# wildjames/lfit_python

Measured on AMD Instinct MI355X. Metric: walker ln_prob evals/sec (300-pt phase, complex BS) at 1/2/4/8 MI355X, higher is better.
Workload: dtype f64

## Files before the change

lfit_python_amd/csrc/lfg.hip:

```cpp
#include <hip/hip_runtime.h>
#include <atomic>
#include <stdint.h>
#include <stdlib.h>

#include <type_traits>

#include "lfg.h"
#include "lfg_device.hpp"
#include "lfg_tables.hpp"

using namespace lfg;

#include "lfg_diag.hpp"

namespace {

constexpr int SETUP_BLOCK = 64;
#ifndef LFG_ELEM_BLOCK
#define LFG_ELEM_BLOCK 64
#endif
constexpr int ELEM_BLOCK = LFG_ELEM_BLOCK;
#ifndef LFG_ELEM_IPL
#define LFG_ELEM_IPL 1
#endif
#ifndef ELEM_MINW
#define ELEM_MINW 4
#endif
constexpr int WT_DISC = 0, WT_TD = NDISC_R, WT_BS = 24, WT_N = WT_BS + NBS;
constexpr int NU_WDD = (NWD + NDISC) / 2, NELU = NU_WDD + NBS;
__device__ __forceinline__ int uitem(int g) { return (g * 37) % NU_WDD; }
__device__ __forceinline__ int uslot(int u) { return (u * 473) % NU_WDD; }
static_assert(NU_WDD == 700 && (37 * 473) % 700 == 1, "sweep permutation inverse");
__device__ __forceinline__ double2 mirror_ab(double2 ab)
{
// ... 422 lines not shown
        G[G_GP_RWD] = rwd;
        G[G_GP_OK] = !ok ? 0.0 : (pend ? 2.0 : (isfinite(B[3]) ? 1.0 : 0.0));
    }
    LFG_CY(3, t, tl);
}

#ifndef LFG_NOLICM_TU
__global__ __launch_bounds__(SETUP_BLOCK) void k_setup(SetupArgs A)
{
    setup_any(A, blockIdx.x * SETUP_BLOCK + threadIdx.x);
}
#endif

#ifdef LFG_COUNT_ITERS
__device__ unsigned long long g_iter_dbg[64];

#endif
constexpr int U_WD = NWD / 2, U_DISC = NDISC / 2, U_BS = NBS, U_DON = NDONOR / 4;
constexpr int NUNIQ = U_WD + U_DISC + U_BS + U_DON;
constexpr int U_MAIN = U_WD + U_DISC + U_DON;

__device__ __forceinline__ int wd_ring_of(int u)
{
    int ir = int(sqrt(u * 0.5));
    if (2 * (ir + 1) * (ir + 1) <= u) ++ir;
    if (2 * ir * ir > u) --ir;
    return ir;
}

__device__ inline double wd_ring_weight(int ir, double ul) { return fma(kWdA[ir], 1.0 - ul, kWdB[ir] * ul); }

template <typename GPtr>
__device__ inline double disc_boundary(int i, GPtr G)
{
    const double rin = G[G_RWD];
    const double r = rin + i * ((G[G_RDISC] - rin) / NDISC_R);
    const double ex = 2.0 - G[G_DEXP];
    return (fabs(ex) < 1e-10) ? log(r) : pow(r, ex) / ex;
}

template <typename GPtr>
__device__ inline double disc_ring_weight(int ir, GPtr G)
{
    return (TWO_PI / NDISC_AZ) * (disc_boundary(ir + 1, G) - disc_boundary(ir, G));
}

template <typename GPtr>
__device__ inline double bs_weight(int j, GPtr G)
{
    const double uk = (j + 0.5) * (G[G_UMAX] / NBS);
// ... 13 lines not shown
    const int* bstatusC;
    const double* priorC;
    const double* qC;
    const double* zfC;
    double* prior;
    double* q;
    double* zf;
    int* bstatus;
    int E, ndim;
    const double* lprior;
    SetupArgs S[2];
    int nspec;
    int nspecblk;
};

struct ElemOut {
    double2* abw;
    double2* abs;
    double* don;
    double* wtd;
    double* wbs;
};

template <typename GPtr>
__device__ __forceinline__ void ring_weight_lane(int rb, GPtr G, double* __restrict__ wtd)
{
    const double P = disc_boundary(rb, G);
    const int lane = int(threadIdx.x) & 63, l0 = lane - rb;
    const double Pn = __shfl(P, min(lane + 1, l0 + NDISC_R), 64);
    const double Pt = __shfl(P, l0 + NDISC_R, 64);
    if (rb < NDISC_R) wtd[rb] = (TWO_PI / NDISC_AZ) * (Pn - P);
    if (rb == 0) wtd[NDISC_R] = TWO_PI * (Pt - P);
}

template <typename GPtr, typename Sink>
__device__ __forceinline__ void element_item_to(int v, GPtr G, Sink& K);

struct MemSink {
    const ElemOut& O;
    __device__ __forceinline__ void mark() {}
    __device__ __forceinline__ void wd_disc(int u, double a, double b) { O.abw[uslot(u)] = make_double2(a, b); }
    __device__ __forceinline__ void spot(int j, double a, double b, double w)
    {
        O.abs[j] = make_double2(a, b);
        O.wbs[j] = w;
    }
    __device__ __forceinline__ void donor(int uu, double vx, double vy, double vz, double cen, double hw)
    {
        double* D = O.don + uu * DON_STRIDE;
        D[0] = vx;
        D[1] = vy;
        D[2] = vz;
        D[3] = cen;
        D[4] = hw;
    }
// ... 67 lines not shown
        const double ig = rsqrt(gx * gx + gy * gy + gz * gz);
        const double nx = gx * ig, ny = gy * ig, nz = gz * ig;
        const double dA = r * r * kDonOmega[it] / (nx * dx + ny * dy + nz * dz);
        const double vx = dA * nx, vy = dA * ny, vz = dA * nz;
        const double srho = s * sqrt(vx * vx + vy * vy);
        const double kap = (srho > 0.0) ? -c * vz / srho : (c * vz > 0.0 ? -2.0 : 2.0);
        const double cen = -atan2(vy, vx) * (1.0 / TWO_PI), hw = acos(fmin(fmax(kap, -1.0), 1.0)) * (1.0 / TWO_PI);
        K.mark();
        K.donor(uu, vx, vy, vz, cen, hw);
        return;
    }

    double Px, Py, Pz;
    if (u < U_WD) {
        const int ir = wd_ring_of(u);
        const double rc = kWdRc[ir], mu0 = kWdMu0[ir];
        const double cp = kWdCos[u], sp = kWdSin[u];
        const double rw = G[G_RWD];
        Px = rw * (-rc * sp * c + mu0 * s);
        Py = rw * (rc * cp);
        Pz = rw * (rc * sp * s + mu0 * c);
    } else if (u < U_WD + U_DISC) {
        const int uu = u - U_WD;
        const int ir = uu / (NDISC_AZ / 2), j = uu - ir * (NDISC_AZ / 2);
        const double rin = G[G_RWD];
        const double rc = rin + (ir + 0.5) * ((G[G_RDISC] - rin) / NDISC_R);
        Px = rc * kDiscCos[j];
        Py = rc * kDiscSin[j];
        Pz = 0.0;
    } else {
        const int j = u - U_MAIN;
        const double uk = (j + 0.5) * (G[G_UMAX] / NBS);
        const double off = G[G_L] * (uk - G[G_UPK]);
        Px = fma(off, G[G_CAZ], G[G_BSX]);
        Py = fma(off, G[G_SAZ], G[G_BSY]);
        Pz = 0.0;
    }
    double a, b;
#ifdef LFG_COUNT_ITERS
    bool fb = false;
    int nit[3] = {0, 0, 0};
    double gs[2] = {0.0, 0.0};
    element_interval_fast(R, Px, Py, Pz, s, c, G[G_RCAL], G[G_REFF], a, b, &fb, nit, gs);
    {
        const int reg = (u < U_WD) ? 0 : (u < U_WD + U_DISC ? 1 : 2);
        unsigned long long* C = g_iter_dbg + reg * 16;
        for (int i = 0; i < 3; ++i) {
// ... 259 lines not shown
        const uint4 r = draw(L.seed, L.step, L.half, 1, w);
        const double lu = log(u53(r.x, r.y));
        if (lu < L.zfac[w] + v - L.lnp_ens[wg]) {
            double* p = L.pos + size_t(wg) * L.ndim;
            const double* qi = L.qprop + size_t(w) * L.ndim;
            for (int d = 0; d < L.ndim; ++d) p[d] = qi[d];
            L.lnp_ens[wg] = v;
            if (L.naccept) L.naccept[wg] += 1;
            if (L.accflag) L.accflag[w] = 1;
        } else if (L.accflag) {
            L.accflag[w] = 0;
        }
    }
}

__device__ inline void finish_walker(const LikeArgs& L, int pair, int tid, bool acc1, const double* sq,
                                     const double* sacc1, int* sflag);

__device__ inline void combine_after(const LikeArgs& L, int pair)
{
    if (L.combine) combine_walker(L, pair / L.E);
}

constexpr int LIKE_THREADS = 512;
constexpr int ACC_LDS = 24;
#ifndef LIKE_MINW
#define LIKE_MINW 4
#endif
constexpr int LIKE_TILE = LIKE_THREADS;
constexpr int LIKE_NC = 2 * LIKE_TILE;
#ifndef LFG_WALK
#define LFG_WALK 2
#endif
constexpr double FX_SCALE = 2305843009213693952.0;
constexpr double FX_INV = 1.0 / FX_SCALE;

struct PhaseIndex {
    const double* v;
    const int* cell;
    int m;
    double t0, ginv;
};

__device__ __forceinline__ int cell_of(const PhaseIndex& X, double v)
{
    const double u = (v - X.t0) * X.ginv;
    return u <= 0.0 ? 0 : (u >= double(LIKE_NC) ? LIKE_NC : int(u));
}

template <bool LE>
__device__ __forceinline__ int count_below(const PhaseIndex& X, double x)
{
    int j = X.cell[cell_of(X, x)];
    const int last = X.m - 1;
    bool adv = false;
#pragma unroll
    for (int k = 0; k < LFG_WALK; ++k) {
        const double vj = X.v[min(j, last)];
        adv = (j <= last) & (LE ? (vj <= x) : (vj < x));
        j += adv ? 1 : 0;
    }
    if (adv)
        while (j <= last && (LE ? (X.v[j] <= x) : (X.v[j] < x))) ++j;
    return j;
}

template <int Q>
__device__ __forceinline__ void count_lt_multi(const PhaseIndex& X, const double (&x)[Q], int (&j)[Q])
{
    const int last = X.m - 1;
#pragma unroll
    for (int q = 0; q < Q; ++q) j[q] = X.cell[cell_of(X, x[q])];
    bool adv[Q];
#pragma unroll
    for (int k = 0; k < LFG_WALK; ++k) {
#pragma unroll
        for (int q = 0; q < Q; ++q) {
            const double vj = X.v[min(j[q], last)];
            adv[q] = (j[q] <= last) & (vj < x[q]);
            j[q] += adv[q] ? 1 : 0;
        }
    }
#pragma unroll
    for (int q = 0; q < Q; ++q)
        if (adv[q])
            while (j[q] <= last && X.v[j[q]] < x[q]) ++j[q];
}

template <int Q>
__device__ __forceinline__ void count_le_back_multi(const double* __restrict__ hi, const double (&x)[Q],
                                                    const int (&J)[Q], int (&out)[Q])
{
    bool back[Q];
#pragma unroll
    for (int q = 0; q < Q; ++q) {
        back[q] = (J[q] > 0) & (hi[max(J[q] - 1, 0)] > x[q]);
        out[q] = J[q] - (back[q] ? 1 : 0);
    }
#pragma unroll
    for (int q = 0; q < Q; ++q)
        if (back[q])
            while (out[q] > 0 && hi[out[q] - 1] > x[q]) --out[q];
}

__device__ __forceinline__ int count_le_back(const double* __restrict__ hi, int J, double x)
{
    const bool back = (J > 0) & (hi[max(J - 1, 0)] > x);
    J -= back ? 1 : 0;
    if (back)
        while (J > 0 && hi[J - 1] > x) --J;
    return J;
}

__device__ __forceinline__ PhaseIndex phase_index(const double* v, const int* cell, int m)
{
    const double span = v[m - 1] - v[0];
    return PhaseIndex{v, cell, m, v[0], span > 0.0 ? LIKE_NC / span : 0.0};
}

__device__ __forceinline__ void build_cells(const double* __restrict__ v, int m, int* __restrict__ cell, int tid)
{
    const PhaseIndex X = phase_index(v, cell, m);
    const double t0 = X.t0, ginv = X.ginv;
    auto ci = [&](double x) {
        const double u = (x - t0) * ginv;
        return u < 0.0 ? -1 : (u >= double(LIKE_NC) ? LIKE_NC : int(u));
    };
    if (tid < m) {
        const int g0 = tid ? ci(v[tid - 1]) : -1, g1 = ci(v[tid]);
        for (int g = g0 + 1; g <= g1; ++g) cell[g] = tid;
        if (tid == m - 1)
            for (int g = g1 + 1; g <= LIKE_NC; ++g) cell[g] = m;
    }
}

__device__ __forceinline__ long long to_fx(double x) { return static_cast<long long>(rint(x * FX_SCALE)); }

__device__ __forceinline__ void fx_add(unsigned long long* acc, int p, long long q)
{
    atomicAdd(acc + p, static_cast<unsigned long long>(q));
}

struct Runs {
    int P1, P2, P3, P4;
};

__device__ __forceinline__ Runs element_runs(double a, double b, const PhaseIndex& X, const double* __restrict__ hi)
{
    Runs R;
    R.P2 = count_below<false>(X, a);
    R.P4 = count_below<false>(X, b);
    R.P1 = count_le_back(hi, R.P2, a);
    R.P3 = count_le_back(hi, R.P4, b);
    return R;
}

__device__ __forceinline__ void apply_runs(const Runs& R, double a, double b, double wn, const PhaseIndex& X,
                                           const double* __restrict__ hi, const double* __restrict__ iw,
                                           unsigned long long* acc)
{
    const int P1 = R.P1, P2 = R.P2, P3 = R.P3, P4 = R.P4;
    int e0 = P4, s1 = P4;
    if (P2 < P3) {
        const long long q = to_fx(wn);
        fx_add(acc, P2, q);
        if (P3 < X.m) fx_add(acc, P3, -q);
        e0 = P2;
        s1 = P3;
    }
    for (int r = 0; r < 2; ++r) {
        const int pe = r ? P4 : e0;
        for (int p = r ? s1 : P1; p < pe; ++p) {
            const double ov = fmin(b, hi[p]) - fmax(a, X.v[p]);
            if (ov > 0.0) {
                const long long q = to_fx(wn * ov * iw[p]);
                fx_add(acc, p, q);
                if (p + 1 < X.m) fx_add(acc, p + 1, -q);
            }
        }
    }
}

template <int NI>
__device__ __forceinline__ void apply_runs_batched(const Runs (&R)[NI], const double (&a)[NI], const double (&b)[NI],
                                                   double wn, const PhaseIndex& X, const double* __restrict__ hi,
                                                   const double* __restrict__ iw, unsigned long long* acc)
{
    constexpr int K = 2;
    const int last = X.m - 1;
    int ps[NI][2], pn[NI][2];
    long long q[NI][2][K];
#pragma unroll
    for (int k = 0; k < NI; ++k) {
        const bool whole = R[k].P2 < R[k].P3;
        const int e0 = whole ? R[k].P2 : R[k].P4, s1 = whole ? R[k].P3 : R[k].P4;
        ps[k][0] = R[k].P1;
        pn[k][0] = e0 - R[k].P1;
        ps[k][1] = s1;
        pn[k][1] = R[k].P4 - s1;
#pragma unroll
        for (int e = 0; e < 2; ++e)
#pragma unroll
            for (int i = 0; i < K; ++i) {
                const int p = min(ps[k][e] + i, last);
                const double ov = fmin(b[k], hi[p]) - fmax(a[k], X.v[p]);
                q[k][e][i] = (i < pn[k][e] && ov > 0.0) ? to_fx(wn * ov * iw[p]) : 0;
            }
    }
    const long long qw = to_fx(wn);
#pragma unroll
    for (int k = 0; k < NI; ++k) {
        if (R[k].P2 < R[k].P3) {
            fx_add(acc, R[k].P2, qw);
            if (R[k].P3 < X.m) fx_add(acc, R[k].P3, -qw);
        }
#pragma unroll
        for (int e = 0; e < 2; ++e)
#pragma unroll
            for (int i = 0; i < K; ++i) {
                const int p = ps[k][e] + i;
                if (q[k][e][i] != 0) {
                    fx_add(acc, p, q[k][e][i]);
                    if (p + 1 < X.m) fx_add(acc, p + 1, -q[k][e][i]);
                }
            }
    }
#pragma unroll
    for (int k = 0; k < NI; ++k)
#pragma unroll
        for (int e = 0; e < 2; ++e)
            for (int p = ps[k][e] + K; p < ps[k][e] + pn[k][e]; ++p) {
                const double ov = fmin(b[k], hi[p]) - fmax(a[k], X.v[p]);
                if (ov > 0.0) {
                    const long long qq = to_fx(wn * ov * iw[p]);
                    fx_add(acc, p, qq);
                    if (p + 1 < X.m) fx_add(acc, p + 1, -qq);
                }
            }
}

__device__ __forceinline__ int uring(int u)
{
    if (u >= U_WD) return NWD_RINGS + (u - U_WD) / (NDISC_AZ / 2);
    int r = int(sqrtf(float(u) * 0.5f));
    r += (2 * (r + 1) * (r + 1) <= u) ? 1 : 0;
    r -= (2 * r * r > u) ? 1 : 0;
    return r;
}

__device__ __forceinline__ long long wave_scan_incl(long long v, int lane)
{
    (void)lane;
    v += dpp64<0x111, 0xf>(v);
    v += dpp64<0x112, 0xf>(v);
    v += dpp64<0x114, 0xf>(v);
    v += dpp64<0x118, 0xf>(v);
    v += dpp64<0x142, 0xa>(v);
    v += dpp64<0x143, 0xc>(v);
    return v;
}

__device__ __forceinline__ long long wave_total(long long v)
{
    v = wave_scan_incl(v, 0);
    const int lo = __builtin_amdgcn_readlane(static_cast<int>(v), 63);
    const int hi = __builtin_amdgcn_readlane(static_cast<int>(v >> 32), 63);
    return (static_cast<long long>(hi) << 32) | static_cast<unsigned>(lo);
}

template <int NA>
// ... 1152 lines not shown
    double2* ab;
    double2* sab;
    double* sbw;
    double* sdq;
    unsigned long long* mk;
    long long tspot, tdon, bx, by, bz;

    __device__ __forceinline__ void mark()
    {
#ifdef LFG_PROFILE_PAIR
        if (mk) *mk = __builtin_amdgcn_s_memrealtime();
#endif
    }
    __device__ __forceinline__ void wd_disc(int u, double a, double b)
    {
#ifdef LFG_ABL_SINK_WD
        return;
#endif
        if (dir) {
            ab[uslot(u)] = make_double2(a, b);
            return;
        }
        if (!(a < b)) return;
        const int ir = uring(u);
        const double wn = (u < U_WD) ? wd_ring_weight(ir, ul) * itwd : swt[ir - NWD_RINGS] * (1.0 / swt[NDISC_R]);
        double q[4] = {a, b, -b, -a};
        int J[4], Jb[4];
        count_lt_multi<4>(XW, q, J);
        count_le_back_multi<4>(hi, q, J, Jb);
        unsigned long long* A = ((lane & 1) ? acc2 : acc)[(u < U_WD) ? 0 : 1];
        const Runs RR[2] = {Runs{Jb[0], J[0], Jb[1], J[1]}, Runs{Jb[2], J[2], Jb[3], J[3]}};
        const double aa[2] = {a, -b}, bb[2] = {b, -a};
        apply_runs_batched<2>(RR, aa, bb, wn, XW, hi, iw, A);
    }
    __device__ __forceinline__ void spot(int j, double a, double b, double w)
    {
        sab[j] = make_double2(a, b);
        sbw[j] = w;
        tspot += to_fx(w * PAIR_SPOT_S);
#ifdef LFG_ABL_SINK_SPOT
        if (false) {
#else
        if (!dir && a < b) {
#endif
            const Runs RR[1] = {element_runs(a, b, XW, hi)};
            const double aa[1] = {a}, bb[1] = {b};
            apply_runs_batched<1>(RR, aa, bb, w * PAIR_SPOT_S, XW, hi, iw, acc[2]);
        }
    }
    __device__ __forceinline__ void donor(int uu, double vx0, double vy0, double vz0, double cen0, double hw0)
    {
        double* D = sdq + uu * DON_STRIDE;
        D[0] = vx0;
        D[1] = vy0;
        D[2] = vz0;
        D[3] = cen0;
        D[4] = hw0;
        long long tn = 0;
        int PA[4][2], QA[4][2];
#pragma unroll
        for (int mr = 0; mr < 4; ++mr) {
            const double vy = (mr & 1) ? -vy0 : vy0, vz = (mr & 2) ? -vz0 : vz0;
            const double cen = (mr & 1) ? -cen0 : cen0;
            const double hw = (mr & 2) ? 0.5 - hw0 : hw0;
            tn += to_fx(fmax(-s * vy + c * vz, 0.0) * PAIR_DON_S);
            PA[mr][0] = QA[mr][0] = PA[mr][1] = QA[mr][1] = 0;
#ifdef LFG_ABL_SINK_DON
            continue;
#endif
            if (dir || !(hw > 0.0)) continue;
// ... 505 lines not shown
        amin[1] = fmin(amin[1], W.part[5][k]); bmax[1] = fmax(bmax[1], W.part[6][k]);
        sa = fmin(sa, W.part[2][k]); sb = fmax(sb, W.part[3][k]); vs += W.part[4][k];
    }
    double t0[2], ginv[2];
    for (int t = 0; t < 2; ++t) {
        t0[t] = amin[t];
        ginv[t] = (bmax[t] > amin[t]) ? LONG_FC / (bmax[t] - amin[t]) : 0.0;
    }
    const double st0 = sa, sginv = (sb > sa) ? TCELLS / (sb - sa) : 0.0;
    constexpr double t0d = -0.5, t1d = 0.5, dginv = TCELLS;
    const double itb = 1.0 / (double(static_cast<long long>(stot[0])) * (FX_INV / PAIR_SPOT_S)), ivs = 1.0 / vs;
    if (tid == 0) {
        for (int t = 0; t < 2; ++t) { W.t0[t] = t0[t]; W.ginv[t] = ginv[t]; W.amin[t] = amin[t]; W.bmax[t] = bmax[t]; }
        W.snorm[0] = itb;
        W.snorm[1] = ivs;
        W.snorm[2] = double(static_cast<long long>(stot[1])) * (FX_INV / PAIR_DON_S);
        W.snorm[3] = vs;
        W.shull[0] = fmin(amin[0], amin[1]); W.shull[1] = fmax(bmax[0], bmax[1]); W.shull[2] = sa; W.shull[3] = sb;
        T.dt0 = t0d; T.dginv = dginv; T.st0 = st0; T.sginv = sginv;
    }
    auto wd_entry = [&](int g, double2& ab, int& t, long long& q) {
        ab = abw[g];
        if (!(ab.x < ab.y)) return false;
        const int u = uitem(g), ir = uring(u);
        t = u < U_WD ? 0 : 1;
        q = to_fx(u < U_WD ? wd_ring_weight(ir, ul) * itwd : swt[ir - NWD_RINGS] * (1.0 / swt[NDISC_R]));
        return true;
    };
    for (int g = tid; g < NU_WDD; g += nt) {
        double2 ab;
        int t;
        long long q;
        if (!wd_entry(g, ab, t, q)) continue;
        (void)q;
        atomicAdd(&W.fend[t][long_cell(ab.x, t0[t], ginv[t])], 1);
        atomicAdd(&W.fend[t][long_cell(ab.y, t0[t], ginv[t])], 1);
    }
    {
        double p0, p1;
        bool in0, in1;
        int v0;
        lane_breakpoints(tid, sdq, sab, t0d, t1d, p0, p1, in0, in1, v0);
        long long c0[3] = {0, 0, 0};
        if (tid >= nt - NDONOR) {
            long long q[3];
            donor_q(sdq, tid - (nt - NDONOR), ivs, q[0], q[1], q[2]);
            for (int k = 0; k < 3; ++k) c0[k] = v0 * q[k];
// ... 215 lines not shown
        for (int k = k0; k < k1; ++k) {
            run += q[k];
            q[k] = run;
        }
    }
    if (tid >= 128 && tid < 128 + U_DON) {
        double* dq = sdq + (tid - 128) * DON_STRIDE;
        const long long q0 = to_fx(dq[0] * ivs), q1 = to_fx(dq[1] * ivs), q2 = to_fx(dq[2] * ivs);
        LongV* dl = reinterpret_cast<LongV*>(dq);
        dl[0] = q0;
        dl[1] = q1;
        dl[2] = q2;
    }
    __syncthreads();
    LONG_TSTAMP(6);
}

template <bool GP, bool FOLD = false, bool LONG = false>
__global__ __launch_bounds__(LIKE_THREADS, LIKE_MINW) void k_pair(PairArgs A)
{
    static_assert(!(GP && LONG), "GP trees keep the one-tile layout or the two kernels");
    const LikeArgs& L = A.L;
    const ElemSpec& X = A.X;
    __shared__ double swt[NDISC_R + 1];
    __shared__ double sbw[NBS];
    __shared__ double2 sab[NBS];
    __shared__ double sdq[U_DON * DON_STRIDE];
    __shared__ double sacc1[3];
    __shared__ TileBufs TA;
    __shared__ double sph[LIKE_TILE];
    __shared__ union PairU_ {
        struct {
            unsigned long long X[2][LIKE_TILE + 1];
            int scp[LIKE_NC + 1];
        } s;
        double2 ab[NU_WDD];
    } SU;
    __shared__ unsigned long long sacc[6][LIKE_TILE + 1];
    __shared__ unsigned long long stot[2];
#if !LFG_PAIR_RUNSCAN
    __shared__ long long spart[6][LIKE_THREADS / 64];
#endif
    __shared__ double red[LIKE_THREADS / 64];
    __shared__ int sflagw[LIKE_THREADS / 64];
    __shared__ int sflag[1];
    __shared__ int sjob;
    __shared__ double sq[ACC_LDS];
// ... 123 lines not shown
        if (tid <= m) {
            for (int i = 0; i < 6; ++i) sacc[i][tid] = 0ull;
            SU.s.X[0][tid] = 0ull;
            SU.s.X[1][tid] = 0ull;
        }
#else
        for (int i = 0; i < 6; ++i) sacc[i][tid] = 0ull;
        SU.s.X[0][tid] = 0ull;
        SU.s.X[1][tid] = 0ull;
#endif
    }
    if (tid == 0) {
#if !LFG_PAIR_RUNSCAN
        if constexpr (!LONG) {
            for (int i = 0; i < 6; ++i) sacc[i][nt] = 0ull;
            SU.s.X[0][nt] = 0ull;
            SU.s.X[1][nt] = 0ull;
        }
#endif
        stot[0] = stot[1] = 0ull;
        sjob = (X.nspec > 0 && pair < 2 * A.nbc) ? 8 : 9;
    }
    PAIR_STAMP(19, tid == 0);
    if (st == ST_OK && wv == 7 && lane <= NDISC_R) ring_weight_lane(lane, Gc, swt);
    __syncthreads();
    PAIR_STAMP(16, tid == 0);

    bool dir = LONG;
    if (!LONG)
        for (int k = 0; k < nw; ++k) dir = dir || sflagw[k] != 0;
    if (own) {
        sy[tid] = L.y[o0 + tid];
        if (!GP) sye[tid] = L.ye[o0 + tid];
        if (GP) {
            const double xp = L.x[o0 + tid], dx = xp - (tid ? L.x[o0 + tid - 1] : xp);
            L.gpx[size_t(pair) * L.N + tid] = exp(-(Gc[G_GP_LAM] * dx));
        }
    }
    const bool pend = GP && st == ST_OK && Gc[G_GP_OK] == 2.0;
    auto fold_rows = [&](int l) {
        const int ns = A.jns, h = L.half, hp = 1 - h, nd = L.ndim, r = (ns + nwk - 1) / nwk;
        for (int f = l; f < r * nd; f += 64) {
            const int k = f / nd, d = f - k * nd, j = w + k * nwk;
            if (j < ns) A.fsnap[size_t(j) * nd + d] = A.fpos[(size_t(h) * ns + j) * nd + d];
        }
        if (A.fv) {
            for (int f = l; f < r * nd; f += 64) {
// ... 87 lines not shown
                                          r1 * (sp * s), s, c, eggleton(R.q), a, b))
                        b = NAN;
                }
            }
            double lo = isnan(b) ? INFINITY : b, hi = isnan(b) ? -INFINITY : b;
            for (int off = DCP_LANES / 2; off > 0; off >>= 1) {
                lo = fmin(lo, __shfl_xor(lo, off, DCP_LANES));
                hi = fmax(hi, __shfl_xor(hi, off, DCP_LANES));
            }
            if (k == 0) {
                ok = ok && lo <= hi;
                const double d = ok ? (Gc[G_GP_DPHI] + (hi - lo)) / 2.0 : NAN;
                double* Gd = const_cast<double*>(L.geo) + size_t(pair) * LFG_NGEO;
                Gd[G_GP_DCP] = d;
                Gd[G_GP_OK] = ok ? 1.0 : 0.0;
                sdcp = d;
            }
        } else if (!pend && tid == 0) {
            sdcp = Gc[G_GP_DCP];
        }
    }
    if (st == ST_OK && m > 0) {
        const double ul = Gc[G_ULIMB];
        const double itwd = 1.0 / (TWO_PI * ((1.0 - ul) * 0.5 + ul / 3.0));
        auto make_sink = [&]() {
            if constexpr (LONG)
                return PairSink{true, lane, PhaseIndex{}, PhaseIndex{}, nullptr, nullptr, nullptr, nullptr, stot, swt,
                                ul, itwd, Gc[G_S], Gc[G_C], Lab, sab, sbw, sdq};
            else
                return PairSink{dir, lane, phase_index(TA.lo, TA.cell, m), phase_index(sph, SU.s.scp, m), TA.hi,
                                TA.iw, sacc, SU.s.X, stot, swt, ul, itwd, Gc[G_S], Gc[G_C], SU.ab, sab, sbw, sdq};
        };
        PairSink K = make_sink();
        auto chunk = [&](int j) {
            const int c = kJobChunk[j - 1];
            constexpr int V_BS = U_WD + U_DISC, V_DON = V_BS + U_BS;
            const int r0 = c < 11 ? 0 : (c < 13 ? V_BS : V_DON), c0 = c < 11 ? 0 : (c < 13 ? 11 : 13);
            const int r1 = c < 11 ? V_BS : (c < 13 ? V_DON : NUNIQ);
            const int v = r0 + (c - c0) * 64 + lane < r1 ? r0 + (c - c0) * 64 + lane : -1;
#ifdef LFG_PROFILE_PAIR
            const bool rec = lane == 0 && blockIdx.x < 4096;
            if (rec) g_pair_j[0][c][blockIdx.x] = __builtin_amdgcn_s_memrealtime();
            K.mk = rec ? &g_pair_j[1][c][blockIdx.x] : nullptr;
#endif
            if (v >= 0) element_item_to(v, Gc, K);
#ifdef LFG_PROFILE_PAIR
            if (rec) g_pair_j[2][c][blockIdx.x] = __builtin_amdgcn_s_memrealtime();
#endif
        };
        auto grab = [&]() {
            int j = 0;
            if (lane == 0) j = atomicAdd(&sjob, 1);
            return __builtin_amdgcn_readfirstlane(j);
        };
// ... 1817 lines not shown
```

lfit_python_amd/csrc/lfg_tables.hpp:

```cpp
#pragma once
#include <hip/hip_runtime.h>
namespace lfg {
__constant__ const double kWdCos[200] = {
    0.70710678118654757, 0.70710678118654735, 0.96592582628906831, 0.70710678118654757,
    0.25881904510252074, 0.2588190451025203, 0.70710678118654735, 0.96592582628906809,
    0.98768834059513777, 0.8910065241883679, 0.70710678118654757, 0.4539904997395468,
    0.15643446504023092, 0.15643446504023067, 0.45399049973954664, 0.70710678118654735,
    0.89100652418836779, 0.98768834059513766, 0.9937122098932426, 0.94388333030836757,
    0.84672419922828412, 0.70710678118654757, 0.53203207651533657, 0.33027906195516732,
    0.11196447610330769, 0.11196447610330768, 0.33027906195516687, 0.53203207651533635,
    0.70710678118654735, 0.84672419922828401, 0.94388333030836746, 0.9937122098932426,
    0.99619469809174555, 0.96592582628906831, 0.90630778703664994, 0.8191520442889918,
    0.70710678118654757, 0.57357643635104616, 0.42261826174069944, 0.25881904510252096,
    0.087155742747658138, 0.087155742747657888, 0.2588190451025203, 0.42261826174069883,
    0.57357643635104605, 0.70710678118654735, 0.81915204428899158, 0.90630778703664971,
    0.96592582628906831, 0.99619469809174555, 0.99745211461025352, 0.97714686597115952,
    0.9369497249997617, 0.87767898956725565, 0.80054124092436041, 0.70710678118654757,
    0.59927766651134695, 0.479248986720057, 0.34946417959909842, 0.21256528955297682,
    0.071339183199232353, 0.071339183199231673, 0.21256528955297679, 0.34946417959909837,
    0.47924898672005678, 0.59927766651134684, 0.70710678118654735, 0.80054124092436019,
    0.87767898956725543, 0.93694972499976192, 0.97714686597115941, 0.99745211461025352,
    0.9981755542233175, 0.98361990694714363, 0.9547208665085456, 0.91189984599209006,
    0.85578127230144752, 0.7871834806090503, 0.70710678118654746, 0.61671887262854319,
    0.51733781417765679, 0.41041280545275693, 0.29750305385520298, 0.18025503781390587,
// ... 94 lines not shown
    0.0070018923404746164, 0.0065458916079624389, 0.0059523977588250079, 0.0051736044474914276,
    0.004101962746066755, 0.0022823141497946139};
__constant__ const unsigned char kWdRingOf[400] = {
    0, 0, 0, 0, 1, 1, 1, 1, 1, 1, 1, 1, 1, 1, 1, 1, 2, 2, 2, 2,
    2, 2, 2, 2, 2, 2, 2, 2, 2, 2, 2, 2, 2, 2, 2, 2, 3, 3, 3, 3,
    3, 3, 3, 3, 3, 3, 3, 3, 3, 3, 3, 3, 3, 3, 3, 3, 3, 3, 3, 3,
    3, 3, 3, 3, 4, 4, 4, 4, 4, 4, 4, 4, 4, 4, 4, 4, 4, 4, 4, 4,
    4, 4, 4, 4, 4, 4, 4, 4, 4, 4, 4, 4, 4, 4, 4, 4, 4, 4, 4, 4,
    5, 5, 5, 5, 5, 5, 5, 5, 5, 5, 5, 5, 5, 5, 5, 5, 5, 5, 5, 5,
    5, 5, 5, 5, 5, 5, 5, 5, 5, 5, 5, 5, 5, 5, 5, 5, 5, 5, 5, 5,
    5, 5, 5, 5, 6, 6, 6, 6, 6, 6, 6, 6, 6, 6, 6, 6, 6, 6, 6, 6,
    6, 6, 6, 6, 6, 6, 6, 6, 6, 6, 6, 6, 6, 6, 6, 6, 6, 6, 6, 6,
    6, 6, 6, 6, 6, 6, 6, 6, 6, 6, 6, 6, 6, 6, 6, 6, 7, 7, 7, 7,
    7, 7, 7, 7, 7, 7, 7, 7, 7, 7, 7, 7, 7, 7, 7, 7, 7, 7, 7, 7,
    7, 7, 7, 7, 7, 7, 7, 7, 7, 7, 7, 7, 7, 7, 7, 7, 7, 7, 7, 7,
    7, 7, 7, 7, 7, 7, 7, 7, 7, 7, 7, 7, 7, 7, 7, 7, 8, 8, 8, 8,
    8, 8, 8, 8, 8, 8, 8, 8, 8, 8, 8, 8, 8, 8, 8, 8, 8, 8, 8, 8,
    8, 8, 8, 8, 8, 8, 8, 8, 8, 8, 8, 8, 8, 8, 8, 8, 8, 8, 8, 8,
    8, 8, 8, 8, 8, 8, 8, 8, 8, 8, 8, 8, 8, 8, 8, 8, 8, 8, 8, 8,
    8, 8, 8, 8, 9, 9, 9, 9, 9, 9, 9, 9, 9, 9, 9, 9, 9, 9, 9, 9,
    9, 9, 9, 9, 9, 9, 9, 9, 9, 9, 9, 9, 9, 9, 9, 9, 9, 9, 9, 9,
    9, 9, 9, 9, 9, 9, 9, 9, 9, 9, 9, 9, 9, 9, 9, 9, 9, 9, 9, 9,
    9, 9, 9, 9, 9, 9, 9, 9, 9, 9, 9, 9, 9, 9, 9, 9, 9, 9, 9, 9};
__constant__ const double kDiscCos[25] = {
    0.99802672842827156, 0.98228725072868872, 0.95105651629515353, 0.90482705246601958,
    0.84432792550201508, 0.77051324277578925, 0.68454710592868862, 0.58778525229247325,
    0.48175367410171516, 0.36812455268467809, 0.24868988716485474, 0.12533323356430448,
    6.123233995736766e-17, -0.12533323356430415, -0.24868988716485485, -0.36812455268467775,
    -0.48175367410171543, -0.58778525229247303, -0.68454710592868873, -0.77051324277578914,
    -0.84432792550201485, -0.90482705246601935, -0.95105651629515353, -0.98228725072868872,
    -0.99802672842827156};
__constant__ const double kDiscSin[25] = {
    0.062790519529313374, 0.1873813145857246, 0.3090169943749474, 0.42577929156507266,
    0.53582679497899666, 0.63742398974868963, 0.72896862742141155, 0.80901699437494734,
    0.87630668004386369, 0.92977648588825135, 0.96858316112863108, 0.99211470131447776,
    1, 0.99211470131447788, 0.96858316112863108, 0.92977648588825146,
    0.87630668004386347, 0.80901699437494745, 0.72896862742141144, 0.63742398974868986,
    0.53582679497899699, 0.42577929156507288, 0.30901699437494751, 0.18738131458572457,
    0.062790519529313582};
__constant__ const double kDonCt[20] = {
    0.99691733373312796, 0.97236992039767656, 0.92387953251128674, 0.85264016435409218,
    0.76040596560003093, 0.64944804833018366, 0.52249856471594891, 0.38268343236508984,
    0.23344536385590547, 0.078459095727844999, -0.078459095727844874, -0.23344536385590534,
    -0.38268343236508973, -0.5224985647159488, -0.64944804833018355, -0.76040596560003093,
    -0.85264016435409218, -0.92387953251128674, -0.97236992039767656, -0.99691733373312796};
__constant__ const double kDonSt[20] = {
// ... 63 lines not shown
```

Before: 15.14 million.

## Merge pair-sink run updates, tabulate ring lookups, precompute phase index constants

Result: faster. 15.54 million (median of 6 runs) (+2.6%).

```diff
diff --git a/lfit_python_amd/csrc/lfg.hip b/lfit_python_amd/csrc/lfg.hip
--- a/lfit_python_amd/csrc/lfg.hip
+++ b/lfit_python_amd/csrc/lfg.hip
@@ -8,8 +8,13 @@
 #include "lfg.h"
 #include "lfg_device.hpp"
 #include "lfg_tables.hpp"
+#include "lfg_sweep.hpp"
 
 using namespace lfg;
+
+#ifndef LFG_PAIR_SINK_MERGE
+#define LFG_PAIR_SINK_MERGE 1
+#endif
 
 #include "lfg_diag.hpp"
 
@@ -478,10 +483,14 @@
 
 __device__ __forceinline__ int wd_ring_of(int u)
 {
+#if LFG_PAIR_SINK_MERGE
+    return kRingOf[u];
+#else
     int ir = int(sqrt(u * 0.5));
     if (2 * (ir + 1) * (ir + 1) <= u) ++ir;
     if (2 * ir * ir > u) --ir;
     return ir;
+#endif
 }
 
 __device__ inline double wd_ring_weight(int ir, double ul) { return fma(kWdA[ir], 1.0 - ul, kWdB[ir] * ul); }
@@ -541,7 +550,7 @@
     double* wbs;
 };
 
-template <typename GPtr>
+template <bool RCP = false, typename GPtr>
 __device__ __forceinline__ void ring_weight_lane(int rb, GPtr G, double* __restrict__ wtd)
 {
     const double P = disc_boundary(rb, G);
@@ -550,6 +559,7 @@
     const double Pt = __shfl(P, l0 + NDISC_R, 64);
     if (rb < NDISC_R) wtd[rb] = (TWO_PI / NDISC_AZ) * (Pn - P);
     if (rb == 0) wtd[NDISC_R] = TWO_PI * (Pt - P);
+    if (RCP && rb == 0) wtd[NDISC_R + 1] = 1.0 / (TWO_PI * (Pt - P));
 }
 
 template <typename GPtr, typename Sink>
@@ -663,7 +673,11 @@
         Pz = rw * (rc * sp * s + mu0 * c);
     } else if (u < U_WD + U_DISC) {
         const int uu = u - U_WD;
+#if LFG_PAIR_SINK_MERGE
+        const int ir = kRingOf[u] - NWD_RINGS, j = uu - ir * (NDISC_AZ / 2);
+#else
         const int ir = uu / (NDISC_AZ / 2), j = uu - ir * (NDISC_AZ / 2);
+#endif
         const double rin = G[G_RWD];
         const double rc = rin + (ir + 0.5) * ((G[G_RDISC] - rin) / NDISC_R);
         Px = rc * kDiscCos[j];
@@ -969,101 +983,10 @@
     if (L.combine) combine_walker(L, pair / L.E);
 }
 
-constexpr int LIKE_THREADS = 512;
 constexpr int ACC_LDS = 24;
 #ifndef LIKE_MINW
 #define LIKE_MINW 4
 #endif
-constexpr int LIKE_TILE = LIKE_THREADS;
-constexpr int LIKE_NC = 2 * LIKE_TILE;
-#ifndef LFG_WALK
-#define LFG_WALK 2
-#endif
-constexpr double FX_SCALE = 2305843009213693952.0;
-constexpr double FX_INV = 1.0 / FX_SCALE;
-
-struct PhaseIndex {
-    const double* v;
-    const int* cell;
-    int m;
-    double t0, ginv;
-};
-
-__device__ __forceinline__ int cell_of(const PhaseIndex& X, double v)
-{
-    const double u = (v - X.t0) * X.ginv;
-    return u <= 0.0 ? 0 : (u >= double(LIKE_NC) ? LIKE_NC : int(u));
-}
-
-template <bool LE>
-__device__ __forceinline__ int count_below(const PhaseIndex& X, double x)
-{
-    int j = X.cell[cell_of(X, x)];
-    const int last = X.m - 1;
-    bool adv = false;
-#pragma unroll
-    for (int k = 0; k < LFG_WALK; ++k) {
-        const double vj = X.v[min(j, last)];
-        adv = (j <= last) & (LE ? (vj <= x) : (vj < x));
-        j += adv ? 1 : 0;
-    }
-    if (adv)
-        while (j <= last && (LE ? (X.v[j] <= x) : (X.v[j] < x))) ++j;
-    return j;
-}
-
-template <int Q>
-__device__ __forceinline__ void count_lt_multi(const PhaseIndex& X, const double (&x)[Q], int (&j)[Q])
-{
-    const int last = X.m - 1;
-#pragma unroll
-    for (int q = 0; q < Q; ++q) j[q] = X.cell[cell_of(X, x[q])];
-    bool adv[Q];
-#pragma unroll
-    for (int k = 0; k < LFG_WALK; ++k) {
-#pragma unroll
-        for (int q = 0; q < Q; ++q) {
-            const double vj = X.v[min(j[q], last)];
-            adv[q] = (j[q] <= last) & (vj < x[q]);
-            j[q] += adv[q] ? 1 : 0;
-        }
-    }
-#pragma unroll
-    for (int q = 0; q < Q; ++q)
-        if (adv[q])
-            while (j[q] <= last && X.v[j[q]] < x[q]) ++j[q];
-}
-
-template <int Q>
-__device__ __forceinline__ void count_le_back_multi(const double* __restrict__ hi, const double (&x)[Q],
-                                                    const int (&J)[Q], int (&out)[Q])
-{
-    bool back[Q];
-#pragma unroll
-    for (int q = 0; q < Q; ++q) {
-        back[q] = (J[q] > 0) & (hi[max(J[q] - 1, 0)] > x[q]);
-        out[q] = J[q] - (back[q] ? 1 : 0);
-    }
-#pragma unroll
-    for (int q = 0; q < Q; ++q)
-        if (back[q])
-            while (out[q] > 0 && hi[out[q] - 1] > x[q]) --out[q];
-}
-
-__device__ __forceinline__ int count_le_back(const double* __restrict__ hi, int J, double x)
-{
-    const bool back = (J > 0) & (hi[max(J - 1, 0)] > x);
-    J -= back ? 1 : 0;
-    if (back)
-        while (J > 0 && hi[J - 1] > x) --J;
-    return J;
-}
-
-__device__ __forceinline__ PhaseIndex phase_index(const double* v, const int* cell, int m)
-{
-    const double span = v[m - 1] - v[0];
-    return PhaseIndex{v, cell, m, v[0], span > 0.0 ? LIKE_NC / span : 0.0};
-}
 
 __device__ __forceinline__ void build_cells(const double* __restrict__ v, int m, int* __restrict__ cell, int tid)
 {
@@ -1081,51 +1004,21 @@
     }
 }
 
-__device__ __forceinline__ long long to_fx(double x) { return static_cast<long long>(rint(x * FX_SCALE)); }
-
 __device__ __forceinline__ void fx_add(unsigned long long* acc, int p, long long q)
 {
     atomicAdd(acc + p, static_cast<unsigned long long>(q));
 }
 
-struct Runs {
-    int P1, P2, P3, P4;
+struct FxAdd {
+    unsigned long long* acc;
+    __device__ __forceinline__ void operator()(int p, long long q) const { fx_add(acc, p, q); }
 };
-
-__device__ __forceinline__ Runs element_runs(double a, double b, const PhaseIndex& X, const double* __restrict__ hi)
-{
-    Runs R;
-    R.P2 = count_below<false>(X, a);
-    R.P4 = count_below<false>(X, b);
-    R.P1 = count_le_back(hi, R.P2, a);
-    R.P3 = count_le_back(hi, R.P4, b);
-    return R;
-}
 
 __device__ __forceinline__ void apply_runs(const Runs& R, double a, double b, double wn, const PhaseIndex& X,
                                            const double* __restrict__ hi, const double* __restrict__ iw,
                                            unsigned long long* acc)
 {
-    const int P1 = R.P1, P2 = R.P2, P3 = R.P3, P4 = R.P4;
-    int e0 = P4, s1 = P4;
-    if (P2 < P3) {
-        const long long q = to_fx(wn);
-        fx_add(acc, P2, q);
-        if (P3 < X.m) fx_add(acc, P3, -q);
-        e0 = P2;
-        s1 = P3;
-    }
-    for (int r = 0; r < 2; ++r) {
-        const int pe = r ? P4 : e0;
-        for (int p = r ? s1 : P1; p < pe; ++p) {
-            const double ov = fmin(b, hi[p]) - fmax(a, X.v[p]);
-            if (ov > 0.0) {
-                const long long q = to_fx(wn * ov * iw[p]);
-                fx_add(acc, p, q);
-                if (p + 1 < X.m) fx_add(acc, p + 1, -q);
-            }
-        }
-    }
+    lfg::apply_runs(R, a, b, wn, X, hi, iw, FxAdd{acc});
 }
 
 template <int NI>
@@ -1133,58 +1026,18 @@
                                                    double wn, const PhaseIndex& X, const double* __restrict__ hi,
                                                    const double* __restrict__ iw, unsigned long long* acc)
 {
-    constexpr int K = 2;
-    const int last = X.m - 1;
-    int ps[NI][2], pn[NI][2];
-    long long q[NI][2][K];
-#pragma unroll
-    for (int k = 0; k < NI; ++k) {
-        const bool whole = R[k].P2 < R[k].P3;
-        const int e0 = whole ? R[k].P2 : R[k].P4, s1 = whole ? R[k].P3 : R[k].P4;
-        ps[k][0] = R[k].P1;
-        pn[k][0] = e0 - R[k].P1;
-        ps[k][1] = s1;
-        pn[k][1] = R[k].P4 - s1;
-#pragma unroll
-        for (int e = 0; e < 2; ++e)
-#pragma unroll
-            for (int i = 0; i < K; ++i) {
-                const int p = min(ps[k][e] + i, last);
-                const double ov = fmin(b[k], hi[p]) - fmax(a[k], X.v[p]);
-                q[k][e][i] = (i < pn[k][e] && ov > 0.0) ? to_fx(wn * ov * iw[p]) : 0;
-            }
-    }
-    const long long qw = to_fx(wn);
-#pragma unroll
-    for (int k = 0; k < NI; ++k) {
-        if (R[k].P2 < R[k].P3) {
-            fx_add(acc, R[k].P2, qw);
-            if (R[k].P3 < X.m) fx_add(acc, R[k].P3, -qw);
-        }
-#pragma unroll
-        for (int e = 0; e < 2; ++e)
-#pragma unroll
-            for (int i = 0; i < K; ++i) {
-                const int p = ps[k][e] + i;
-                if (q[k][e][i] != 0) {
-                    fx_add(acc, p, q[k][e][i]);
-                    if (p + 1 < X.m) fx_add(acc, p + 1, -q[k][e][i]);
-                }
-            }
-    }
-#pragma unroll
-    for (int k = 0; k < NI; ++k)
-#pragma unroll
-        for (int e = 0; e < 2; ++e)
-            for (int p = ps[k][e] + K; p < ps[k][e] + pn[k][e]; ++p) {
-                const double ov = fmin(b[k], hi[p]) - fmax(a[k], X.v[p]);
-                if (ov > 0.0) {
-                    const long long qq = to_fx(wn * ov * iw[p]);
-                    fx_add(acc, p, qq);
-                    if (p + 1 < X.m) fx_add(acc, p + 1, -qq);
-                }
-            }
-}
+    lfg::apply_runs_batched<NI>(R, a, b, wn, X, hi, iw, FxAdd{acc});
+}
+
+#if LFG_PAIR_SINK_MERGE
+template <int NI>
+__device__ __forceinline__ void apply_runs_merged(const Runs (&R)[NI], const double (&a)[NI], const double (&b)[NI],
+                                                  double wn, const PhaseIndex& X, const double* __restrict__ hi,
+                                                  const double* __restrict__ iw, unsigned long long* acc)
+{
+    lfg::apply_runs_merged<NI>(R, a, b, wn, X, hi, iw, FxAdd{acc}, [](bool slow) { return __any(slow) != 0; });
+}
+#endif
 
 __device__ __forceinline__ int uring(int u)
 {
@@ -1193,6 +1046,15 @@
     r += (2 * (r + 1) * (r + 1) <= u) ? 1 : 0;
     r -= (2 * r * r > u) ? 1 : 0;
     return r;
+}
+
+__device__ __forceinline__ int pair_ring(int u)
+{
+#if LFG_PAIR_SINK_MERGE
+    return kRingOf[u];
+#else
+    return uring(u);
+#endif
 }
 
 __device__ __forceinline__ long long wave_scan_incl(long long v, int lane)
@@ -2391,8 +2253,12 @@
             return;
         }
         if (!(a < b)) return;
-        const int ir = uring(u);
+        const int ir = pair_ring(u);
+#if LFG_PAIR_SINK_MERGE
+        const double wn = (u < U_WD) ? wd_ring_weight(ir, ul) * itwd : swt[ir - NWD_RINGS] * swt[NDISC_R + 1];
+#else
         const double wn = (u < U_WD) ? wd_ring_weight(ir, ul) * itwd : swt[ir - NWD_RINGS] * (1.0 / swt[NDISC_R]);
+#endif
         double q[4] = {a, b, -b, -a};
         int J[4], Jb[4];
         count_lt_multi<4>(XW, q, J);
@@ -2400,7 +2266,11 @@
         unsigned long long* A = ((lane & 1) ? acc2 : acc)[(u < U_WD) ? 0 : 1];
         const Runs RR[2] = {Runs{Jb[0], J[0], Jb[1], J[1]}, Runs{Jb[2], J[2], Jb[3], J[3]}};
         const double aa[2] = {a, -b}, bb[2] = {b, -a};
+#if LFG_PAIR_SINK_MERGE
+        apply_runs_merged<2>(RR, aa, bb, wn, XW, hi, iw, A);
+#else
         apply_runs_batched<2>(RR, aa, bb, wn, XW, hi, iw, A);
+#endif
     }
     __device__ __forceinline__ void spot(int j, double a, double b, double w)
     {
@@ -2414,7 +2284,11 @@
 #endif
             const Runs RR[1] = {element_runs(a, b, XW, hi)};
             const double aa[1] = {a}, bb[1] = {b};
+#if LFG_PAIR_SINK_MERGE
+            apply_runs_merged<1>(RR, aa, bb, w * PAIR_SPOT_S, XW, hi, iw, acc[2]);
+#else
             apply_runs_batched<1>(RR, aa, bb, w * PAIR_SPOT_S, XW, hi, iw, acc[2]);
+#endif
         }
     }
     __device__ __forceinline__ void donor(int uu, double vx0, double vy0, double vz0, double cen0, double hw0)
@@ -2966,7 +2840,7 @@
     auto wd_entry = [&](int g, double2& ab, int& t, long long& q) {
         ab = abw[g];
         if (!(ab.x < ab.y)) return false;
-        const int u = uitem(g), ir = uring(u);
+        const int u = uitem(g), ir = pair_ring(u);
         t = u < U_WD ? 0 : 1;
         q = to_fx(u < U_WD ? wd_ring_weight(ir, ul) * itwd : swt[ir - NWD_RINGS] * (1.0 / swt[NDISC_R]));
         return true;
@@ -3228,7 +3102,12 @@
     static_assert(!(GP && LONG), "GP trees keep the one-tile layout or the two kernels");
     const LikeArgs& L = A.L;
     const ElemSpec& X = A.X;
+#if LFG_PAIR_SINK_MERGE
+    __shared__ double swt[NDISC_R + (LONG ? 1 : 2)];
+    __shared__ double skc[5];
+#else
     __shared__ double swt[NDISC_R + 1];
+#endif
     __shared__ double sbw[NBS];
     __shared__ double2 sab[NBS];
     __shared__ double sdq[U_DON * DON_STRIDE];
@@ -3398,7 +3277,26 @@
         sjob = (X.nspec > 0 && pair < 2 * A.nbc) ? 8 : 9;
     }
     PAIR_STAMP(19, tid == 0);
+#if LFG_PAIR_SINK_MERGE
+    if (st == ST_OK && wv == 7 && lane <= NDISC_R) ring_weight_lane<!LONG>(lane, Gc, swt);
+    if (!LONG && st == ST_OK && m > 0 && wv == 6 && lane < 3) {
+        double ph0, lo0, hi0, hw0, ph1, lo1, hi1, hw1;
+        pair_window(xw_0, ww_0, phi0, ph0, lo0, hi0, hw0);
+        pair_window(xw_1, ww_1, phi0, ph1, lo1, hi1, hw1);
+        const double ulk = Gc[G_ULIMB];
+        const double v0 = lane == 1 ? lo0 : ph0, span = (lane == 1 ? lo1 : ph1) - v0;
+        const double num = lane ? double(LIKE_NC) : 1.0;
+        const double den = lane ? span : TWO_PI * ((1.0 - ulk) * 0.5 + ulk / 3.0);
+        const double quo = num / den;
+        if (lane == 0) skc[0] = quo;
+        else {
+            skc[2 * lane - 1] = v0;
+            skc[2 * lane] = span > 0.0 ? quo : 0.0;
+        }
+    }
+#else
     if (st == ST_OK && wv == 7 && lane <= NDISC_R) ring_weight_lane(lane, Gc, swt);
+#endif
     __syncthreads();
     PAIR_STAMP(16, tid == 0);
 
@@ -3532,14 +3430,25 @@
     }
     if (st == ST_OK && m > 0) {
         const double ul = Gc[G_ULIMB];
+#if LFG_PAIR_SINK_MERGE
+        const double itwd = LONG ? 1.0 / (TWO_PI * ((1.0 - ul) * 0.5 + ul / 3.0)) : skc[0];
+#else
         const double itwd = 1.0 / (TWO_PI * ((1.0 - ul) * 0.5 + ul / 3.0));
+#endif
         auto make_sink = [&]() {
             if constexpr (LONG)
                 return PairSink{true, lane, PhaseIndex{}, PhaseIndex{}, nullptr, nullptr, nullptr, nullptr, stot, swt,
                                 ul, itwd, Gc[G_S], Gc[G_C], Lab, sab, sbw, sdq};
+#if LFG_PAIR_SINK_MERGE
+            else
+                return PairSink{dir, lane, PhaseIndex{TA.lo, TA.cell, m, skc[1], skc[2]},
+                                PhaseIndex{sph, SU.s.scp, m, skc[3], skc[4]}, TA.hi,
+                                TA.iw, sacc, SU.s.X, stot, swt, ul, itwd, Gc[G_S], Gc[G_C], SU.ab, sab, sbw, sdq};
+#else
             else
                 return PairSink{dir, lane, phase_index(TA.lo, TA.cell, m), phase_index(sph, SU.s.scp, m), TA.hi,
                                 TA.iw, sacc, SU.s.X, stot, swt, ul, itwd, Gc[G_S], Gc[G_C], SU.ab, sab, sbw, sdq};
+#endif
         };
         PairSink K = make_sink();
         auto chunk = [&](int j) {
diff --git a/lfit_python_amd/csrc/lfg_sweep.hpp b/lfit_python_amd/csrc/lfg_sweep.hpp
--- /dev/null
+++ b/lfit_python_amd/csrc/lfg_sweep.hpp
@@ -0,0 +1,248 @@
+#pragma once
+#include <hip/hip_runtime.h>
+#include <math.h>
+
+namespace lfg {
+
+constexpr int LIKE_THREADS = 512;
+constexpr int LIKE_TILE = LIKE_THREADS;
+constexpr int LIKE_NC = 2 * LIKE_TILE;
+#ifndef LFG_WALK
+#define LFG_WALK 2
+#endif
+constexpr double FX_SCALE = 2305843009213693952.0;
+constexpr double FX_INV = 1.0 / FX_SCALE;
+
+struct PhaseIndex {
+    const double* v;
+    const int* cell;
+    int m;
+    double t0, ginv;
+};
+
+__device__ __forceinline__ int cell_of(const PhaseIndex& X, double v)
+{
+    const double u = (v - X.t0) * X.ginv;
+    return u <= 0.0 ? 0 : (u >= double(LIKE_NC) ? LIKE_NC : int(u));
+}
+
+template <bool LE>
+__device__ __forceinline__ int count_below(const PhaseIndex& X, double x)
+{
+    int j = X.cell[cell_of(X, x)];
+    const int last = X.m - 1;
+    bool adv = false;
+#pragma unroll
+    for (int k = 0; k < LFG_WALK; ++k) {
+        const double vj = X.v[min(j, last)];
+        adv = (j <= last) & (LE ? (vj <= x) : (vj < x));
+        j += adv ? 1 : 0;
+    }
+    if (adv)
+        while (j <= last && (LE ? (X.v[j] <= x) : (X.v[j] < x))) ++j;
+    return j;
+}
+
+template <int Q>
+__device__ __forceinline__ void count_lt_multi(const PhaseIndex& X, const double (&x)[Q], int (&j)[Q])
+{
+    const int last = X.m - 1;
+#pragma unroll
+    for (int q = 0; q < Q; ++q) j[q] = X.cell[cell_of(X, x[q])];
+    bool adv[Q];
+#pragma unroll
+    for (int k = 0; k < LFG_WALK; ++k) {
+#pragma unroll
+        for (int q = 0; q < Q; ++q) {
+            const double vj = X.v[min(j[q], last)];
+            adv[q] = (j[q] <= last) & (vj < x[q]);
+            j[q] += adv[q] ? 1 : 0;
+        }
+    }
+#pragma unroll
+    for (int q = 0; q < Q; ++q)
+        if (adv[q])
+            while (j[q] <= last && X.v[j[q]] < x[q]) ++j[q];
+}
+
+template <int Q>
+__device__ __forceinline__ void count_le_back_multi(const double* __restrict__ hi, const double (&x)[Q],
+                                                    const int (&J)[Q], int (&out)[Q])
+{
+    bool back[Q];
+#pragma unroll
+    for (int q = 0; q < Q; ++q) {
+        back[q] = (J[q] > 0) & (hi[max(J[q] - 1, 0)] > x[q]);
+        out[q] = J[q] - (back[q] ? 1 : 0);
+    }
+#pragma unroll
+    for (int q = 0; q < Q; ++q)
+        if (back[q])
+            while (out[q] > 0 && hi[out[q] - 1] > x[q]) --out[q];
+}
+
+__device__ __forceinline__ int count_le_back(const double* __restrict__ hi, int J, double x)
+{
+    const bool back = (J > 0) & (hi[max(J - 1, 0)] > x);
+    J -= back ? 1 : 0;
+    if (back)
+        while (J > 0 && hi[J - 1] > x) --J;
+    return J;
+}
+
+__device__ __forceinline__ PhaseIndex phase_index(const double* v, const int* cell, int m)
+{
+    const double span = v[m - 1] - v[0];
+    return PhaseIndex{v, cell, m, v[0], span > 0.0 ? LIKE_NC / span : 0.0};
+}
+
+__device__ __forceinline__ long long to_fx(double x) { return static_cast<long long>(rint(x * FX_SCALE)); }
+
+struct Runs {
+    int P1, P2, P3, P4;
+};
+
+__device__ __forceinline__ Runs element_runs(double a, double b, const PhaseIndex& X, const double* __restrict__ hi)
+{
+    Runs R;
+    R.P2 = count_below<false>(X, a);
+    R.P4 = count_below<false>(X, b);
+    R.P1 = count_le_back(hi, R.P2, a);
+    R.P3 = count_le_back(hi, R.P4, b);
+    return R;
+}
+
+template <class Add>
+__device__ __forceinline__ void apply_runs(const Runs& R, double a, double b, double wn, const PhaseIndex& X,
+                                           const double* __restrict__ hi, const double* __restrict__ iw, Add add)
+{
+    const int P1 = R.P1, P2 = R.P2, P3 = R.P3, P4 = R.P4;
+    int e0 = P4, s1 = P4;
+    if (P2 < P3) {
+        const long long q = to_fx(wn);
+        add(P2, q);
+        if (P3 < X.m) add(P3, -q);
+        e0 = P2;
+        s1 = P3;
+    }
+    for (int r = 0; r < 2; ++r) {
+        const int pe = r ? P4 : e0;
+        for (int p = r ? s1 : P1; p < pe; ++p) {
+            const double ov = fmin(b, hi[p]) - fmax(a, X.v[p]);
+            if (ov > 0.0) {
+                const long long q = to_fx(wn * ov * iw[p]);
+                add(p, q);
+                if (p + 1 < X.m) add(p + 1, -q);
+            }
+        }
+    }
+}
+
+template <int NI, class Add>
+__device__ __forceinline__ void apply_runs_batched(const Runs (&R)[NI], const double (&a)[NI], const double (&b)[NI],
+                                                   double wn, const PhaseIndex& X, const double* __restrict__ hi,
+                                                   const double* __restrict__ iw, Add add)
+{
+    constexpr int K = 2;
+    const int last = X.m - 1;
+    int ps[NI][2], pn[NI][2];
+    long long q[NI][2][K];
+#pragma unroll
+    for (int k = 0; k < NI; ++k) {
+        const bool whole = R[k].P2 < R[k].P3;
+        const int e0 = whole ? R[k].P2 : R[k].P4, s1 = whole ? R[k].P3 : R[k].P4;
+        ps[k][0] = R[k].P1;
+        pn[k][0] = e0 - R[k].P1;
+        ps[k][1] = s1;
+        pn[k][1] = R[k].P4 - s1;
+#pragma unroll
+        for (int e = 0; e < 2; ++e)
+#pragma unroll
+            for (int i = 0; i < K; ++i) {
+                const int p = min(ps[k][e] + i, last);
+                const double ov = fmin(b[k], hi[p]) - fmax(a[k], X.v[p]);
+                q[k][e][i] = (i < pn[k][e] && ov > 0.0) ? to_fx(wn * ov * iw[p]) : 0;
+            }
+    }
+    const long long qw = to_fx(wn);
+#pragma unroll
+    for (int k = 0; k < NI; ++k) {
+        if (R[k].P2 < R[k].P3) {
+            add(R[k].P2, qw);
+            if (R[k].P3 < X.m) add(R[k].P3, -qw);
+        }
+#pragma unroll
+        for (int e = 0; e < 2; ++e)
+#pragma unroll
+            for (int i = 0; i < K; ++i) {
+                const int p = ps[k][e] + i;
+                if (q[k][e][i] != 0) {
+                    add(p, q[k][e][i]);
+                    if (p + 1 < X.m) add(p + 1, -q[k][e][i]);
+                }
+            }
+    }
+#pragma unroll
+    for (int k = 0; k < NI; ++k)
+#pragma unroll
+        for (int e = 0; e < 2; ++e)
+            for (int p = ps[k][e] + K; p < ps[k][e] + pn[k][e]; ++p) {
+                const double ov = fmin(b[k], hi[p]) - fmax(a[k], X.v[p]);
+                if (ov > 0.0) {
+                    const long long qq = to_fx(wn * ov * iw[p]);
+                    add(p, qq);
+                    if (p + 1 < X.m) add(p + 1, -qq);
+                }
+            }
+}
+
+template <int NI, class Add, class Vote>
+__device__ __forceinline__ void apply_runs_merged(const Runs (&R)[NI], const double (&a)[NI], const double (&b)[NI],
+                                                  double wn, const PhaseIndex& X, const double* __restrict__ hi,
+                                                  const double* __restrict__ iw, Add add, Vote any_lane)
+{
+    bool slow = false;
+#pragma unroll
+    for (int k = 0; k < NI; ++k) {
+        const bool whole = R[k].P2 < R[k].P3;
+        const int cut = min(R[k].P1 + 1, R[k].P4);
+        const int e0 = whole ? R[k].P2 : cut, s1 = whole ? R[k].P3 : cut;
+        slow = slow | (e0 - R[k].P1 > 1) | (R[k].P4 - s1 > 1);
+    }
+    if (any_lane(slow)) {
+        apply_runs_batched<NI>(R, a, b, wn, X, hi, iw, add);
+        return;
+    }
+    const int last = X.m - 1;
+    int ps[NI][2];
+    long long s[NI][2][2];
+    const long long qw = to_fx(wn);
+#pragma unroll
+    for (int k = 0; k < NI; ++k) {
+        const bool whole = R[k].P2 < R[k].P3;
+        const int cut = min(R[k].P1 + 1, R[k].P4);
+        const int e0 = whole ? R[k].P2 : cut, s1 = whole ? R[k].P3 : cut;
+        ps[k][0] = R[k].P1;
+        ps[k][1] = s1;
+        const int pn[2] = {e0 - R[k].P1, R[k].P4 - s1};
+#pragma unroll
+        for (int e = 0; e < 2; ++e) {
+            const int p = min(ps[k][e], last);
+            const double ov = fmin(b[k], hi[p]) - fmax(a[k], X.v[p]);
+            const long long q = (pn[e] > 0 && ov > 0.0) ? to_fx(wn * ov * iw[p]) : 0;
+            const long long w0 = !whole ? 0 : (e ? -qw : (pn[0] == 0 ? qw : 0));
+            const long long w1 = (whole && e == 0 && pn[0] == 1) ? qw : 0;
+            s[k][e][0] = q + w0;
+            s[k][e][1] = w1 - q;
+        }
+    }
+#pragma unroll
+    for (int k = 0; k < NI; ++k)
+#pragma unroll
+        for (int e = 0; e < 2; ++e)
+#pragma unroll
+            for (int i = 0; i < 2; ++i)
+                if (s[k][e][i] != 0 && ps[k][e] + i < X.m) add(ps[k][e] + i, s[k][e][i]);
+}
+
+}
diff --git a/lfit_python_amd/csrc/lfg_tables.hpp b/lfit_python_amd/csrc/lfg_tables.hpp
--- a/lfit_python_amd/csrc/lfg_tables.hpp
+++ b/lfit_python_amd/csrc/lfg_tables.hpp
@@ -140,6 +140,35 @@
     9, 9, 9, 9, 9, 9, 9, 9, 9, 9, 9, 9, 9, 9, 9, 9, 9, 9, 9, 9,
     9, 9, 9, 9, 9, 9, 9, 9, 9, 9, 9, 9, 9, 9, 9, 9, 9, 9, 9, 9,
     9, 9, 9, 9, 9, 9, 9, 9, 9, 9, 9, 9, 9, 9, 9, 9, 9, 9, 9, 9};
+__constant__ const unsigned char kRingOf[700] = {
+    0, 0, 1, 1, 1, 1, 1, 1, 2, 2, 2, 2, 2, 2, 2, 2, 2, 2, 3, 3, 3, 3, 3, 3, 3,
+    3, 3, 3, 3, 3, 3, 3, 4, 4, 4, 4, 4, 4, 4, 4, 4, 4, 4, 4, 4, 4, 4, 4, 4, 4,
+    5, 5, 5, 5, 5, 5, 5, 5, 5, 5, 5, 5, 5, 5, 5, 5, 5, 5, 5, 5, 5, 5, 6, 6, 6,
+    6, 6, 6, 6, 6, 6, 6, 6, 6, 6, 6, 6, 6, 6, 6, 6, 6, 6, 6, 6, 6, 6, 6, 7, 7,
+    7, 7, 7, 7, 7, 7, 7, 7, 7, 7, 7, 7, 7, 7, 7, 7, 7, 7, 7, 7, 7, 7, 7, 7, 7,
+    7, 7, 7, 8, 8, 8, 8, 8, 8, 8, 8, 8, 8, 8, 8, 8, 8, 8, 8, 8, 8, 8, 8, 8, 8,
+    8, 8, 8, 8, 8, 8, 8, 8, 8, 8, 8, 8, 9, 9, 9, 9, 9, 9, 9, 9, 9, 9, 9, 9, 9,
+    9, 9, 9, 9, 9, 9, 9, 9, 9, 9, 9, 9, 9, 9, 9, 9, 9, 9, 9, 9, 9, 9, 9, 9, 9,
+    10, 10, 10, 10, 10, 10, 10, 10, 10, 10, 10, 10, 10, 10, 10, 10, 10, 10, 10, 10, 10, 10, 10, 10, 10,
+    11, 11, 11, 11, 11, 11, 11, 11, 11, 11, 11, 11, 11, 11, 11, 11, 11, 11, 11, 11, 11, 11, 11, 11, 11,
+    12, 12, 12, 12, 12, 12, 12, 12, 12, 12, 12, 12, 12, 12, 12, 12, 12, 12, 12, 12, 12, 12, 12, 12, 12,
+    13, 13, 13, 13, 13, 13, 13, 13, 13, 13, 13, 13, 13, 13, 13, 13, 13, 13, 13, 13, 13, 13, 13, 13, 13,
+    14, 14, 14, 14, 14, 14, 14, 14, 14, 14, 14, 14, 14, 14, 14, 14, 14, 14, 14, 14, 14, 14, 14, 14, 14,
+    15, 15, 15, 15, 15, 15, 15, 15, 15, 15, 15, 15, 15, 15, 15, 15, 15, 15, 15, 15, 15, 15, 15, 15, 15,
+    16, 16, 16, 16, 16, 16, 16, 16, 16, 16, 16, 16, 16, 16, 16, 16, 16, 16, 16, 16, 16, 16, 16, 16, 16,
+    17, 17, 17, 17, 17, 17, 17, 17, 17, 17, 17, 17, 17, 17, 17, 17, 17, 17, 17, 17, 17, 17, 17, 17, 17,
+    18, 18, 18, 18, 18, 18, 18, 18, 18, 18, 18, 18, 18, 18, 18, 18, 18, 18, 18, 18, 18, 18, 18, 18, 18,
+    19, 19, 19, 19, 19, 19, 19, 19, 19, 19, 19, 19, 19, 19, 19, 19, 19, 19, 19, 19, 19, 19, 19, 19, 19,
+    20, 20, 20, 20, 20, 20, 20, 20, 20, 20, 20, 20, 20, 20, 20, 20, 20, 20, 20, 20, 20, 20, 20, 20, 20,
+    21, 21, 21, 21, 21, 21, 21, 21, 21, 21, 21, 21, 21, 21, 21, 21, 21, 21, 21, 21, 21, 21, 21, 21, 21,
+    22, 22, 22, 22, 22, 22, 22, 22, 22, 22, 22, 22, 22, 22, 22, 22, 22, 22, 22, 22, 22, 22, 22, 22, 22,
+    23, 23, 23, 23, 23, 23, 23, 23, 23, 23, 23, 23, 23, 23, 23, 23, 23, 23, 23, 23, 23, 23, 23, 23, 23,
+    24, 24, 24, 24, 24, 24, 24, 24, 24, 24, 24, 24, 24, 24, 24, 24, 24, 24, 24, 24, 24, 24, 24, 24, 24,
+    25, 25, 25, 25, 25, 25, 25, 25, 25, 25, 25, 25, 25, 25, 25, 25, 25, 25, 25, 25, 25, 25, 25, 25, 25,
+    26, 26, 26, 26, 26, 26, 26, 26, 26, 26, 26, 26, 26, 26, 26, 26, 26, 26, 26, 26, 26, 26, 26, 26, 26,
+    27, 27, 27, 27, 27, 27, 27, 27, 27, 27, 27, 27, 27, 27, 27, 27, 27, 27, 27, 27, 27, 27, 27, 27, 27,
+    28, 28, 28, 28, 28, 28, 28, 28, 28, 28, 28, 28, 28, 28, 28, 28, 28, 28, 28, 28, 28, 28, 28, 28, 28,
+    29, 29, 29, 29, 29, 29, 29, 29, 29, 29, 29, 29, 29, 29, 29, 29, 29, 29, 29, 29, 29, 29, 29, 29, 29};
 __constant__ const double kDiscCos[25] = {
     0.99802672842827156, 0.98228725072868872, 0.95105651629515353, 0.90482705246601958,
     0.84432792550201508, 0.77051324277578925, 0.68454710592868862, 0.58778525229247325,
```
